# Chen-Suyi/PointRegGPT

Hardware: AMD Instinct MI355X
Metric: generated point-cloud pairs/sec (node), 128x128 depth, 1000-step DDNM (higher is better)
Workload: dtype bf16; 1 GPU; configs[2]: full pipeline (SE(3) z-buffer reproject + MaskUnet + DDNM sampler + MaskUnet + f64 unproject); batch_per_gpu=64, image_size=128, transitions=1000, sampler=ancestral-ddnm, unet_dim=64, streams=2, parallelism=scene-sharded x1, no collectives, hipgraph=one captured transition (U-Net + update), replayed per step

## Files before the change

### pointreggpt_amd/csrc/attn_fused.hip

```cpp
#include <atomic>
#include <cstdlib>
#include <type_traits>

#include "blocks.h"

namespace prg {

typedef __attribute__((ext_vector_type(8))) __bf16 bf16x8;
typedef __attribute__((ext_vector_type(16))) float f32x16;
typedef __attribute__((ext_vector_type(2))) float f32x2;

namespace {

constexpr int kTP = 64;
constexpr int kHid = 128;
constexpr int kTilesPerBlock = 8;
constexpr int kLaCtxTpb = 8, kLaOutTpb = 8;
__host__ __device__ inline int la_tpb(int ntiles) {
  const int t = ntiles / 8;
  return t < 1 ? 1 : (t > kLaCtxTpb ? kLaCtxTpb : t);
}
__host__ __device__ inline int la_out_tpb(int ntiles) {
  const int t = ntiles / 8;
  return t < 1 ? 1 : (t > kLaOutTpb ? kLaOutTpb : t);
}
constexpr int kLdO = kHid + 8;
constexpr float kLnEps = 1e-5f;

__device__ inline uint32_t pack2(float a, float b) {
  typedef __attribute__((ext_vector_type(2))) __bf16 bf16x2;
  bf16x2 v = {(__bf16)a, (__bf16)b};
  return __builtin_bit_cast(uint32_t, v);
}
__device__ inline float bf_lo(uint32_t w) { return __uint_as_float(w << 16); }
__device__ inline float bf_hi(uint32_t w) { return __uint_as_float(w & 0xffff0000u); }
__device__ inline float fast_exp(float x) { return __builtin_amdgcn_exp2f(x * 1.4426950408889634f); }

template <int C>
struct Geo {
  static constexpr int LDW = C + 8;
  static constexpr int VPT = C / 32;
  static constexpr int KK = C / 16;
};

__device__ inline float quad_sum(float v) {
  v += __builtin_bit_cast(float, __builtin_amdgcn_mov_dpp(__builtin_bit_cast(int, v), 0xB1, 0xF, 0xF, true));
  v += __builtin_bit_cast(float, __builtin_amdgcn_mov_dpp(__builtin_bit_cast(int, v), 0x4E, 0xF, 0xF, true));
  return v;
}

template <int C>
struct XTile {
  uint4 v[Geo<C>::VPT];
  __device__ inline void load(const bf16_t* x, int64_t pix0, int valid) {
    const int row = threadIdx.x >> 2, part = threadIdx.x & 3;
#pragma unroll
    for (int i = 0; i < Geo<C>::VPT; ++i)
      v[i] = row < valid ? *reinterpret_cast<const uint4*>(x + (pix0 + row) * C + (part + 4 * i) * 8) : make_uint4(0, 0, 0, 0);
  }
  __device__ inline void normalize_to(__bf16* xn) const {
    const int row = threadIdx.x >> 2, part = threadIdx.x & 3;
    float f[Geo<C>::VPT][8];
    float s = 0.0f;
#pragma unroll
    for (int i = 0; i < Geo<C>::VPT; ++i) {
      const uint32_t w[4] = {v[i].x, v[i].y, v[i].z, v[i].w};
#pragma unroll
      for (int j = 0; j < 4; ++j) {
        f[i][2 * j] = bf_lo(w[j]);
        f[i][2 * j + 1] = bf_hi(w[j]);
        s += f[i][2 * j] + f[i][2 * j + 1];
      }
    }
    s = quad_sum(s);
    const float mean = s * (1.0f / C);
    float q = 0.0f;
#pragma unroll
    for (int i = 0; i < Geo<C>::VPT; ++i)
#pragma unroll
      for (int j = 0; j < 8; ++j) {
        f[i][j] -= mean;
        q = fmaf(f[i][j], f[i][j], q);
      }
    q = quad_sum(q);
    const float rstd = __builtin_amdgcn_rsqf(q * (1.0f / C) + kLnEps);
#pragma unroll
    for (int i = 0; i < Geo<C>::VPT; ++i) {
      uint4 o;
      o.x = pack2(f[i][0] * rstd, f[i][1] * rstd);
      o.y = pack2(f[i][2] * rstd, f[i][3] * rstd);
      o.z = pack2(f[i][4] * rstd, f[i][5] * rstd);
      o.w = pack2(f[i][6] * rstd, f[i][7] * rstd);
      *reinterpret_cast<uint4*>(xn + row * Geo<C>::LDW + (part + 4 * i) * 8) = o;
    }
  }
};

template <int COLS, int LD>
__device__ inline void stage_rows(__bf16* dst, const bf16_t* src, int nrows) {
  constexpr int VR = COLS / 8;
  for (int i = threadIdx.x; i < nrows * VR; i += 256) {
    const int r = i / VR, v = i - r * VR;
    *reinterpret_cast<uint4*>(dst + r * LD + v * 8) = *reinterpret_cast<const uint4*>(src + (size_t)r * COLS + v * 8);
  }
}

__device__ inline bf16x8 frag(const __bf16* rows, int ld, int l31, int hi, int kk) {
  return *reinterpret_cast<const bf16x8*>(rows + l31 * ld + kk * 16 + hi * 8);
}

template <int COLS>
__device__ inline void load_wfrags(bf16x8 (&w)[COLS / 16], const bf16_t* mat, int r0, int l31, int hi) {
#pragma unroll
  for (int kk = 0; kk < COLS / 16; ++kk)
    w[kk] = *reinterpret_cast<const bf16x8*>(mat + (size_t)(r0 + l31) * COLS + kk * 16 + hi * 8);
}

__device__ inline f32x16 zero16() {
  f32x16 z;
#pragma unroll
  for (int e = 0; e < 16; ++e) z[e] = 0.0f;
  return z;
}

template <int C>
__global__ __launch_bounds__(256) void la_kmax_fused_kernel(const bf16_t* __restrict__ x, const bf16_t* __restrict__ wqkv,
                                                            float* __restrict__ pmax, int N, int nslab) {
  using G = Geo<C>;
  extern __shared__ __attribute__((aligned(16))) char smem[];
  __bf16* xn = reinterpret_cast<__bf16*>(smem);
  const int b = blockIdx.y, slab = blockIdx.x;
  const int wave = threadIdx.x >> 6, lane = threadIdx.x & 63, l31 = lane & 31, hi = lane >> 5;
  const int ntiles = (N + kTP - 1) / kTP;
  const int tpb = la_tpb(ntiles), t0 = slab * tpb, t1 = min(t0 + tpb, ntiles);
  bf16x8 wk[G::KK];
  load_wfrags<C>(wk, wqkv, kHid + 32 * wave, l31, hi);
  float m = -INFINITY;
  XTile<C> xt;
  if (t0 < t1) xt.load(x, (int64_t)b * N + (int64_t)t0 * kTP, min(kTP, N - t0 * kTP));
  for (int t = t0; t < t1; ++t) {
    xt.normalize_to(xn);
    __syncthreads();
    if (t + 1 < t1) xt.load(x, (int64_t)b * N + (int64_t)(t + 1) * kTP, min(kTP, N - (t + 1) * kTP));
    f32x16 acc[2] = {zero16(), zero16()};
#pragma unroll
    for (int kk = 0; kk < G::KK; ++kk) {
#pragma unroll
      for (int pt = 0; pt < 2; ++pt)
        acc[pt] = __builtin_amdgcn_mfma_f32_32x32x16_bf16(frag(xn + pt * 32 * G::LDW, G::LDW, l31, hi, kk), wk[kk], acc[pt], 0, 0, 0);
    }
    const int valid = min(kTP, N - t * kTP);
#pragma unroll
    for (int pt = 0; pt < 2; ++pt)
#pragma unroll
      for (int r = 0; r < 16; ++r) {
        const int px = pt * 32 + (r & 3) + 8 * (r >> 2) + 4 * hi;
        if (px < valid) m = fmaxf(m, acc[pt][r]);
      }
    __syncthreads();
  }
  m = fmaxf(m, __shfl_xor(m, 32, 64));
  if (hi == 0) pmax[((size_t)b * nslab + slab) * kHid + 32 * wave + l31] = m;
}

template <int C, bool PSUM_MFMA, bool KSTAT>
__global__ __launch_bounds__(256, C == 64 ? 3 : (C == 128 ? 2 : 1)) void la_ctx_fused_kernel(const bf16_t* __restrict__ x, const bf16_t* __restrict__ wqkv,
                                                           const float* __restrict__ pmax, float* __restrict__ ctxp,
                                                           float* __restrict__ sump, int N, int nslab) {
  using G = Geo<C>;
  extern __shared__ __attribute__((aligned(16))) char smem[];
  __bf16* xn = reinterpret_cast<__bf16*>(smem);
  const int b = blockIdx.y, slab = blockIdx.x;
  const int wave = threadIdx.x >> 6, lane = threadIdx.x & 63, l31 = lane & 31, hi = lane >> 5;
  const int ntiles = (N + kTP - 1) / kTP;
  const int tpb = la_tpb(ntiles), t0 = slab * tpb, t1 = min(t0 + tpb, ntiles);
  bf16x8 wk[G::KK], wv[G::KK];
  load_wfrags<C>(wk, wqkv, kHid + 32 * wave, l31, hi);
  load_wfrags<C>(wv, wqkv, 2 * kHid + 32 * wave, l31, hi);
  f32x16 kinit0 = zero16();
  if constexpr (!KSTAT) {
    float m = -INFINITY;
    for (int s2 = 0; s2 < nslab; ++s2) m = fmaxf(m, pmax[((size_t)b * nslab + s2) * kHid + 32 * wave + l31]);
#pragma unroll
    for (int e = 0; e < 16; ++e) kinit0[e] = -m;
  }
  f32x16 ctx = zero16();
  f32x16 psum = zero16();
  float ssum = 0.0f;
  bf16x8 ones;
#pragma unroll
  for (int e = 0; e < 8; ++e) ones[e] = (__bf16)1.0f;
  XTile<C> xt;
  if (t0 < t1) xt.load(x, (int64_t)b * N + (int64_t)t0 * kTP, min(kTP, N - t0 * kTP));
  for (int t = t0; t < t1; ++t) {
    xt.normalize_to(xn);
    __syncthreads();
    if (t + 1 < t1) xt.load(x, (int64_t)b * N + (int64_t)(t + 1) * kTP, min(kTP, N - (t + 1) * kTP));
    const int valid = min(kTP, N - t * kTP);
    auto half = [&](const int pt, auto full_c) {
      constexpr bool FULL = decltype(full_c)::value;
      f32x16 k1, v1;
#pragma unroll
      for (int kk = 0; kk < G::KK; ++kk) {
        const bf16x8 xf = frag(xn + pt * 32 * G::LDW, G::LDW, l31, hi, kk);
        k1 = __builtin_amdgcn_mfma_f32_32x32x16_bf16(xf, wk[kk], kk == 0 ? (KSTAT ? zero16() : kinit0) : k1, 0, 0, 0);
        v1 = __builtin_amdgcn_mfma_f32_32x32x16_bf16(xf, wv[kk], kk == 0 ? zero16() : v1, 0, 0, 0);
      }
#pragma unroll
      for (int i = 0; i < 2; ++i) {
        bf16x8 pa, vb;
#pragma unroll
        for (int s2 = 0; s2 < 8; ++s2) {
          const int r = 8 * i + s2;
          float pe = __builtin_amdgcn_exp2f(k1[r]);
          if constexpr (!FULL) pe = (pt * 32 + (r & 3) + 8 * (r >> 2) + 4 * hi) < valid ? pe : 0.0f;
          if constexpr (!PSUM_MFMA) ssum += pe;
          pa[s2] = (__bf16)pe;
          vb[s2] = (__bf16)v1[r];
        }
        ctx = __builtin_amdgcn_mfma_f32_32x32x16_bf16(pa, vb, ctx, 0, 0, 0);
        if constexpr (PSUM_MFMA) psum = __builtin_amdgcn_mfma_f32_32x32x16_bf16(pa, ones, psum, 0, 0, 0);
      }
    };
    if (valid == kTP) {
      half(0, std::true_type{});
      half(1, std::true_type{});
    } else {
      half(0, std::false_type{});
      half(1, std::false_type{});
    }
    __syncthreads();
  }
  const size_t ph = ((size_t)b * 4 + wave) * nslab + slab;
  if constexpr (PSUM_MFMA) {
    if (l31 == 0) {
#pragma unroll
      for (int r = 0; r < 16; ++r) sump[ph * 32 + (r & 3) + 8 * (r >> 2) + 4 * hi] = psum[r];
    }
  } else {
    ssum += __shfl_xor(ssum, 32, 64);
    if (hi == 0) sump[ph * 32 + l31] = ssum;
  }
#pragma unroll
  for (int r = 0; r < 16; ++r) ctxp[ph * 1024 + ((r & 3) + 8 * (r >> 2) + 4 * hi) * 32 + l31] = ctx[r];
}

__global__ __launch_bounds__(256) void la_fin_fused_kernel(const float* __restrict__ ctxp, const float* __restrict__ sump,
                                                           bf16_t* __restrict__ ctxT, int N, int nslab) {
  const int h = blockIdx.x, b = blockIdx.y;
  const size_t ph = ((size_t)b * 4 + h) * nslab;
  const float scale = 0.17677669529663687f / (float)N;
  for (int idx = threadIdx.x; idx < 1024; idx += 256) {
    const int d = idx >> 5, e = idx & 31;
    float c = 0.0f, s = 0.0f;
    int s2 = 0;
    for (; s2 + 8 <= nslab; s2 += 8) {
      float cv[8], sv[8];
#pragma unroll
      for (int u = 0; u < 8; ++u) {
        cv[u] = ctxp[(ph + s2 + u) * 1024 + idx];
        sv[u] = sump[(ph + s2 + u) * 32 + d];
      }
#pragma unroll
      for (int u = 0; u < 8; ++u) {
        c += cv[u];
        s += sv[u];
      }
    }
    for (; s2 < nslab; ++s2) {
      c += ctxp[(ph + s2) * 1024 + idx];
      s += sump[(ph + s2) * 32 + d];
    }
    const int slot = (d >> 4) * 16 + ((d >> 2) & 1) * 8 + ((d >> 3) & 1) * 4 + (d & 3);
    ctxT[((size_t)b * 4 + h) * 1024 + e * 32 + slot] = f32_to_bf16(c / s * scale);
  }
}

template <int C, bool QSTAT>
__global__ __launch_bounds__(256, C == 64 ? 3 : (C == 128 ? 2 : 1)) void la_out_fused_kernel(const bf16_t* __restrict__ x, const bf16_t* __restrict__ wqkv,
                                                           const bf16_t* __restrict__ wout, const float* __restrict__ bias,
                                                           const float* __restrict__ out_g, const bf16_t* __restrict__ ctxT,
                                                           bf16_t* __restrict__ out, int N, const float* __restrict__ qshift) {
  using G = Geo<C>;
  constexpr int RT = C / 32;
  constexpr int NA = RT / 2;
  constexpr int NR = RT > 4 ? RT / 4 : 1;
  constexpr int RTL = RT > 4 ? RT : 4;
  extern __shared__ __attribute__((aligned(16))) char smem[];
  __bf16* xn = reinterpret_cast<__bf16*>(smem);
  __bf16* ot = xn + kTP * G::LDW;
  float* lnb = reinterpret_cast<float*>(ot + kTP * kLdO);
  __bf16* yt = reinterpret_cast<__bf16*>(lnb + kTP * RTL * 2);
  float* bias_l = reinterpret_cast<float*>(yt + kTP * G::LDW);
  float* outg_l = bias_l + C;
  if (threadIdx.x < C) {
    bias_l[threadIdx.x] = bias[threadIdx.x];
    outg_l[threadIdx.x] = out_g[threadIdx.x];
  }
  const int b = blockIdx.y, slab = blockIdx.x;
  const int wave = threadIdx.x >> 6, lane = threadIdx.x & 63, l31 = lane & 31, hi = lane >> 5;
  const int ntiles = (N + kTP - 1) / kTP;
  const int tpb = la_out_tpb(ntiles), t0 = slab * tpb, t1 = min(t0 + tpb, ntiles);
  bf16x8 wq[G::KK];
  load_wfrags<C>(wq, wqkv, 32 * wave, l31, hi);
  bf16x8 ca[2];
#pragma unroll
  for (int i = 0; i < 2; ++i)
    ca[i] = *reinterpret_cast<const bf16x8*>(ctxT + (((size_t)b * 4 + wave) * 32 + l31) * 32 + i * 16 + hi * 8);
  int yrt[NA], ypt[NA];
#pragma unroll
  for (int a = 0; a < NA; ++a) {
    if (RT == 2) { yrt[a] = wave & 1; ypt[a] = wave >> 1; }
    else if (RT <= 4) { yrt[a] = wave; ypt[a] = a; }
    else { yrt[a] = wave * NR + (a >> 1); ypt[a] = a & 1; }
  }
  bf16x8 wo[NR][kHid / 16];
#pragma unroll
  for (int r = 0; r < NR; ++r) load_wfrags<kHid>(wo[r], wout, yrt[RT > 4 ? 2 * r : 0] * 32, l31, hi);
  XTile<C> xt;
  if (t0 < t1) xt.load(x, (int64_t)b * N + (int64_t)t0 * kTP, min(kTP, N - t0 * kTP));
  for (int t = t0; t < t1; ++t) {
    asm volatile("" ::: "memory");
    const XTile<C> xraw = xt;
    const int valid = min(kTP, N - t * kTP);
    xt.normalize_to(xn);
    __syncthreads();
    if (t + 1 < t1) xt.load(x, (int64_t)b * N + (int64_t)(t + 1) * kTP, min(kTP, N - (t + 1) * kTP));
    constexpr bool qstat = QSTAT;
    f32x16 qa[2];
#pragma unroll
    for (int kk = 0; kk < G::KK; ++kk) {
#pragma unroll
      for (int pt = 0; pt < 2; ++pt)
        qa[pt] = __builtin_amdgcn_mfma_f32_32x32x16_bf16(wq[kk], frag(xn + pt * 32 * G::LDW, G::LDW, l31, hi, kk),
                                                         kk == 0 ? zero16() : qa[pt], 0, 0, 0);
    }
#pragma unroll
    for (int pt = 0; pt < 2; ++pt) {
      f32x16 oa = zero16();
      if constexpr (qstat) {
        f32x16 sa = zero16();
        bf16x8 ones;
#pragma unroll
        for (int e = 0; e < 8; ++e) ones[e] = (__bf16)1.0f;
#pragma unroll
        for (int i = 0; i < 2; ++i) {
          bf16x8 qb;
#pragma unroll
          for (int s2 = 0; s2 < 8; ++s2) qb[s2] = (__bf16)__builtin_amdgcn_exp2f(qa[pt][8 * i + s2]);
          oa = __builtin_amdgcn_mfma_f32_32x32x16_bf16(ca[i], qb, oa, 0, 0, 0);
          sa = __builtin_amdgcn_mfma_f32_32x32x16_bf16(ones, qb, sa, 0, 0, 0);
        }
        const float inv = __builtin_amdgcn_rcpf(sa[0]);
        const f32x2 inv2 = {inv, inv};
#pragma unroll
        for (int r = 0; r < 16; r += 2) {
          const f32x2 o2 = f32x2{oa[r], oa[r + 1]} * inv2;
          oa[r] = o2[0];
          oa[r + 1] = o2[1];
        }
      } else {
        float mx = qa[pt][0];
#pragma unroll
        for (int r = 1; r < 16; ++r) mx = fmaxf(mx, qa[pt][r]);
        mx = fmaxf(mx, __shfl_xor(mx, 32, 64));
        float sm = 0.0f;
#pragma unroll
        for (int r = 0; r < 16; ++r) {
          qa[pt][r] = __builtin_amdgcn_exp2f(qa[pt][r] - mx);
          sm += qa[pt][r];
        }
        sm += __shfl_xor(sm, 32, 64);
        const float inv = 1.0f / sm;
#pragma unroll
        for (int i = 0; i < 2; ++i) {
          bf16x8 qb;
#pragma unroll
          for (int s2 = 0; s2 < 8; ++s2) qb[s2] = (__bf16)(qa[pt][8 * i + s2] * inv);
          oa = __builtin_amdgcn_mfma_f32_32x32x16_bf16(ca[i], qb, oa, 0, 0, 0);
        }
// ... 7 lines not shown
        *reinterpret_cast<uint2*>(ot + px * kLdO + 32 * wave + 8 * g4 + 4 * hi) = w;
      }
    }
    __syncthreads();
    f32x16 ya[NA];
#pragma unroll
    for (int a = 0; a < NA; ++a) ya[a] = zero16();
#pragma unroll
    for (int kk = 0; kk < kHid / 16; ++kk) {
#pragma unroll
      for (int a = 0; a < NA; ++a)
        ya[a] = __builtin_amdgcn_mfma_f32_32x32x16_bf16(wo[RT > 4 ? (a >> 1) : 0][kk],
                                                        frag(ot + ypt[a] * 32 * kLdO, kLdO, l31, hi, kk), ya[a], 0, 0, 0);
    }
#pragma unroll
    for (int a = 0; a < NA; ++a) {
      float s1 = 0.0f, s2 = 0.0f;
#pragma unroll
      for (int r = 0; r < 16; ++r) {
        const int c = yrt[a] * 32 + (r & 3) + 8 * (r >> 2) + 4 * hi;
        ya[a][r] += bias_l[c];
        s1 += ya[a][r];
        s2 = fmaf(ya[a][r], ya[a][r], s2);
      }
      const auto sw = __builtin_amdgcn_permlane32_swap(__builtin_bit_cast(unsigned, s1), __builtin_bit_cast(unsigned, s2), false, false);
      const float tot = __builtin_bit_cast(float, (unsigned)sw[0]) + __builtin_bit_cast(float, (unsigned)sw[1]);
      lnb[((ypt[a] * 32 + l31) * RTL + yrt[a]) * 2 + hi] = tot;
    }
    __syncthreads();
#pragma unroll
    for (int a = 0; a < NA; ++a) {
      const int px = ypt[a] * 32 + l31;
      float s1 = 0.0f, s2 = 0.0f;
#pragma unroll
      for (int rt = 0; rt < RT; ++rt) {
        s1 += lnb[(px * RTL + rt) * 2];
        s2 += lnb[(px * RTL + rt) * 2 + 1];
      }
      const float mean = s1 * (1.0f / C);
      const float rstd = __builtin_amdgcn_rsqf(fmaxf(s2 * (1.0f / C) - mean * mean, 0.0f) + kLnEps);
#pragma unroll
      for (int g4 = 0; g4 < 4; ++g4) {
        const int c0 = yrt[a] * 32 + 8 * g4 + 4 * hi;
        const float4 gg = *reinterpret_cast<const float4*>(outg_l + c0);
        uint2 w;
        w.x = pack2((ya[a][4 * g4] - mean) * rstd * gg.x, (ya[a][4 * g4 + 1] - mean) * rstd * gg.y);
        w.y = pack2((ya[a][4 * g4 + 2] - mean) * rstd * gg.z, (ya[a][4 * g4 + 3] - mean) * rstd * gg.w);
        *reinterpret_cast<uint2*>(yt + px * G::LDW + c0) = w;
      }
    }
    __syncthreads();
    {
      const int row = threadIdx.x >> 2, part = threadIdx.x & 3;
      if (row < valid) {
#pragma unroll
        for (int i = 0; i < G::VPT; ++i) {
          const uint4 yv = *reinterpret_cast<const uint4*>(yt + row * G::LDW + (part + 4 * i) * 8);
          const uint4 xv = xraw.v[i];
          uint4 o;
          o.x = pack2(bf_lo(yv.x) + bf_lo(xv.x), bf_hi(yv.x) + bf_hi(xv.x));
          o.y = pack2(bf_lo(yv.y) + bf_lo(xv.y), bf_hi(yv.y) + bf_hi(xv.y));
          o.z = pack2(bf_lo(yv.z) + bf_lo(xv.z), bf_hi(yv.z) + bf_hi(xv.z));
          o.w = pack2(bf_lo(yv.w) + bf_lo(xv.w), bf_hi(yv.w) + bf_hi(xv.w));
          *reinterpret_cast<uint4*>(out + ((int64_t)b * N + (int64_t)t * kTP + row) * C + (part + 4 * i) * 8) = o;
        }
      }
    }
  }
}

template <int NT>
__global__ __launch_bounds__(256) void full_attn_mfma_kernel(const bf16_t* __restrict__ qkv, bf16_t* __restrict__ out) {
  constexpr int N = 32 * NT, LDK = 40, LDV = N + 8;
  __shared__ __attribute__((aligned(16))) __bf16 Ks[N * LDK];
  __shared__ __attribute__((aligned(16))) __bf16 Vt[32 * LDV];
  const int h = blockIdx.x, b = blockIdx.y, tid = threadIdx.x;
  const int wave = tid >> 6, lane = tid & 63, l31 = lane & 31, hi = lane >> 5;
  const bf16_t* base = qkv + (size_t)b * N * 384;
  for (int i = tid; i < N * 4; i += 256) {
    const int key = i >> 2, u = i & 3;
    *reinterpret_cast<uint4*>(Ks + key * LDK + u * 8) =
        *reinterpret_cast<const uint4*>(base + (size_t)key * 384 + 128 + h * 32 + u * 8);
    const uint4 vv = *reinterpret_cast<const uint4*>(base + (size_t)key * 384 + 256 + h * 32 + u * 8);
    const int d = key & 31;
    const int pos = (key & ~31) + (d >> 4) * 16 + ((d >> 2) & 1) * 8 + ((d >> 3) & 1) * 4 + (d & 3);
    const uint32_t w[4] = {vv.x, vv.y, vv.z, vv.w};
#pragma unroll
    for (int j = 0; j < 4; ++j) {
      reinterpret_cast<uint16_t*>(Vt)[(u * 8 + 2 * j) * LDV + pos] = (uint16_t)(w[j] & 0xffffu);
      reinterpret_cast<uint16_t*>(Vt)[(u * 8 + 2 * j + 1) * LDV + pos] = (uint16_t)(w[j] >> 16);
    }
  }
  __syncthreads();
  for (int qt = wave; qt < NT; qt += 4) {
    const bf16_t* qp = base + (size_t)(qt * 32 + l31) * 384 + h * 32 + hi * 8;
    const bf16x8 q0 = *reinterpret_cast<const bf16x8*>(qp), q1 = *reinterpret_cast<const bf16x8*>(qp + 16);
    f32x16 sacc[NT];
    float m = -INFINITY;
#pragma unroll
    for (int kt = 0; kt < NT; ++kt) {
      sacc[kt] = zero16();
      sacc[kt] = __builtin_amdgcn_mfma_f32_32x32x16_bf16(frag(Ks + kt * 32 * LDK, LDK, l31, hi, 0), q0, sacc[kt], 0, 0, 0);
      sacc[kt] = __builtin_amdgcn_mfma_f32_32x32x16_bf16(frag(Ks + kt * 32 * LDK, LDK, l31, hi, 1), q1, sacc[kt], 0, 0, 0);
#pragma unroll
      for (int r = 0; r < 16; ++r) {
        sacc[kt][r] *= 0.17677669529663687f;
        m = fmaxf(m, sacc[kt][r]);
      }
    }
    m = fmaxf(m, __shfl_xor(m, 32, 64));
    float l = 0.0f;
    f32x16 oacc = zero16();
#pragma unroll
    for (int kt = 0; kt < NT; ++kt) {
#pragma unroll
      for (int i = 0; i < 2; ++i) {
        bf16x8 pb;
#pragma unroll
        for (int s2 = 0; s2 < 8; ++s2) {
          const float pv = fast_exp(sacc[kt][8 * i + s2] - m);
// ... 39 lines not shown
    for (int j = 0; j < 4; ++j) {
      reinterpret_cast<uint16_t*>(Vt)[(u * 8 + 2 * j) * LDV + pos] = (uint16_t)(w[j] & 0xffffu);
      reinterpret_cast<uint16_t*>(Vt)[(u * 8 + 2 * j + 1) * LDV + pos] = (uint16_t)(w[j] >> 16);
    }
  }
  __syncthreads();
  for (int qt = qs * 4 + wave; qt < NT; qt += 4 * QS) {
    const bf16_t* qp = base + (size_t)(qt * 32 + l31) * 384 + h * 32 + hi * 8;
    const bf16x8 q0 = *reinterpret_cast<const bf16x8*>(qp), q1 = *reinterpret_cast<const bf16x8*>(qp + 16);
    float m = -INFINITY;
#pragma unroll 2
    for (int kt = 0; kt < NT; ++kt) {
      f32x16 sa = zero16();
      sa = __builtin_amdgcn_mfma_f32_32x32x16_bf16(frag(Ks + kt * 32 * LDK, LDK, l31, hi, 0), q0, sa, 0, 0, 0);
      sa = __builtin_amdgcn_mfma_f32_32x32x16_bf16(frag(Ks + kt * 32 * LDK, LDK, l31, hi, 1), q1, sa, 0, 0, 0);
#pragma unroll
      for (int r = 0; r < 16; ++r) m = fmaxf(m, sa[r] * 0.17677669529663687f);
    }
    m = fmaxf(m, __shfl_xor(m, 32, 64));
    float l = 0.0f;
    f32x16 oacc = zero16();
#pragma unroll 2
    for (int kt = 0; kt < NT; ++kt) {
      f32x16 sa = zero16();
      sa = __builtin_amdgcn_mfma_f32_32x32x16_bf16(frag(Ks + kt * 32 * LDK, LDK, l31, hi, 0), q0, sa, 0, 0, 0);
      sa = __builtin_amdgcn_mfma_f32_32x32x16_bf16(frag(Ks + kt * 32 * LDK, LDK, l31, hi, 1), q1, sa, 0, 0, 0);
#pragma unroll
      for (int i = 0; i < 2; ++i) {
        bf16x8 pb;
#pragma unroll
        for (int s2 = 0; s2 < 8; ++s2) {
          const float pv = fast_exp(sa[8 * i + s2] * 0.17677669529663687f - m);
          l += pv;
          pb[s2] = (__bf16)pv;
        }
        oacc = __builtin_amdgcn_mfma_f32_32x32x16_bf16(
            *reinterpret_cast<const bf16x8*>(Vt + l31 * LDV + kt * 32 + i * 16 + hi * 8), pb, oacc, 0, 0, 0);
      }
    }
    l += __shfl_xor(l, 32, 64);
    const float inv = 1.0f / l;
    bf16_t* op = out + ((size_t)b * N + qt * 32 + l31) * 128 + h * 32 + 4 * hi;
#pragma unroll
    for (int g4 = 0; g4 < 4; ++g4) {
      uint2 w;
      w.x = pack2(oacc[4 * g4] * inv, oacc[4 * g4 + 1] * inv);
      w.y = pack2(oacc[4 * g4 + 2] * inv, oacc[4 * g4 + 3] * inv);
      *reinterpret_cast<uint2*>(op + 8 * g4) = w;
    }
  }
}

template <int C>
size_t lds_kmax() { return (size_t)kTP * Geo<C>::LDW * 2; }
template <int C>
size_t lds_out() { return (size_t)2 * kTP * Geo<C>::LDW * 2 + (size_t)kTP * kLdO * 2 + (size_t)kTP * (C / 32 > 4 ? C / 32 : 4) * 2 * 4 + (size_t)2 * C * 4; }

template <typename K>
int set_lds(K kernel, size_t bytes) {
  hipError_t e = hipFuncSetAttribute(reinterpret_cast<const void*>(kernel), hipFuncAttributeMaxDynamicSharedMemorySize, (int)bytes);
  if (e != hipSuccess) return fail(PRG_E_HIP, std::string("hipFuncSetAttribute(fused attention): ") + hipGetErrorString(e));
  return PRG_OK;
}

int la_slabs(int N) { const int nt = ceil_div(N, kTP); return ceil_div(nt, la_tpb(nt)); }
int tail_slabs(int N) { return ceil_div(ceil_div(N, kTP), kTilesPerBlock); }

constexpr int kTailDepth = 2;
template <int CIN, int COUT>
__global__ __launch_bounds__(256, COUT == 64 ? 3 : 2) void resblock_tail_fused_kernel(
    const bf16_t* __restrict__ h, const float* __restrict__ A, const float* __restrict__ Bc, const bf16_t* __restrict__ s0, int C0,
    const bf16_t* __restrict__ s1, int C1, const bf16_t* __restrict__ wres, const float* __restrict__ bres, bf16_t* __restrict__ out,
    int N, const float* __restrict__ head_w, const float* __restrict__ head_b, float* __restrict__ head_out, int head_sigmoid,
    const GnFold fold) {
  constexpr int LDX = CIN + 8, LDH = COUT + 8;
  constexpr int RT = COUT / 32, NA = RT / 2;
  constexpr int XV = CIN / 32, HV = COUT / 32;
  extern __shared__ __attribute__((aligned(16))) char smem[];
  __bf16* xs = reinterpret_cast<__bf16*>(smem);
  __bf16* hs = xs + kTP * LDX;
  float* cf = reinterpret_cast<float*>(hs + kTP * LDH);
  const int b = blockIdx.y, slab = blockIdx.x;
  const int wave = threadIdx.x >> 6, lane = threadIdx.x & 63, l31 = lane & 31, hi = lane >> 5;
  const int row = threadIdx.x >> 2, part = threadIdx.x & 3;
  const int ntiles = (N + kTP - 1) / kTP;
  const int t0 = slab * kTilesPerBlock, t1 = min(t0 + kTilesPerBlock, ntiles);
  const int yrt = RT == 2 ? (wave & 1) : wave;
  int ypt[NA];
#pragma unroll
  for (int a = 0; a < NA; ++a) ypt[a] = RT == 2 ? (wave >> 1) : a;
  bf16x8 wr[CIN / 16];
  load_wfrags<CIN>(wr, wres, yrt * 32, l31, hi);
  if (threadIdx.x < COUT) {
    const int c = threadIdx.x;
    float a, bb;
    if (fold.acc) {
      float mean, rstd;
      gn_fold_stats(fold, b, c / fold.cpg, mean, rstd);
      a = rstd * fold.P[(size_t)b * fold.pq_stride + c];
      bb = fmaf(-mean, a, fold.Q[(size_t)b * fold.pq_stride + c]);
    } else {
      a = A[(size_t)b * COUT + c];
      bb = Bc[(size_t)b * COUT + c];
    }
    cf[c] = a;
    cf[COUT + c] = bb;
    cf[2 * COUT + c] = bres[c];
// ... 64 lines not shown
          acc = fmaf(bf_hi(q[j]), w[2 * j + 1], acc);
        }
      }
      acc += __shfl_xor(acc, 1, 64);
      acc += __shfl_xor(acc, 2, 64);
      if (part == 0 && row < valid) {
        const float y = acc + hb;
        head_out[(int64_t)b * N + (int64_t)t * kTP + row] = head_sigmoid ? 1.0f / (1.0f + expf(-y)) : y;
      }
    } else if (row < valid) {
#pragma unroll
      for (int i = 0; i < HV; ++i)
        *reinterpret_cast<uint4*>(out + ((int64_t)b * N + (int64_t)t * kTP + row) * COUT + (part + 4 * i) * 8) =
            *reinterpret_cast<const uint4*>(hs + row * LDH + (part + 4 * i) * 8);
    }
    __syncthreads();
  };
  load_tile(ta, t0);
  load_tile(tb, t0 + 1);
  for (int t = t0; t < t1; t += kTailDepth) {
    do_tile(ta, t);
    do_tile(tb, t + 1);
  }
}

template <int CIN, int COUT>
int launch_tail(const bf16_t* h, const float* A, const float* Bc, const bf16_t* s0, int C0, const bf16_t* s1, int C1,
                const bf16_t* wres, const float* bres, bf16_t* out, int B, int N, hipStream_t s, const GnFold& fold,
                const float* head_w = nullptr, const float* head_b = nullptr, float* head_out = nullptr, int head_sigmoid = 0) {
  const size_t lds = (size_t)kTP * (CIN + 8 + COUT + 8) * 2 + (size_t)4 * COUT * 4;
  static DeviceOnce attr;
  if (!attr.done()) {
    int rc = set_lds(&resblock_tail_fused_kernel<CIN, COUT>, lds);
    if (rc) return rc;
    attr.mark();
  }
  resblock_tail_fused_kernel<CIN, COUT><<<dim3(tail_slabs(N), B), 256, lds, s>>>(h, A, Bc, s0, C0, s1, C1, wres, bres, out, N, head_w, head_b,
                                                                                 head_out, head_sigmoid, fold);
  PRG_LAUNCH_CHECK();
  return PRG_OK;
}


template <int C>
constexpr bool kPsumDefault = C >= 128;

template <int C>
int launch_c(const bf16_t* x, const bf16_t* wqkv, const bf16_t* wout, const float* bias, const float* out_g, bf16_t* out,
             float* ws, int B, int N, const float* kshift, hipStream_t s, int psum_override) {
  static DeviceOnce attr;
  if (!attr.done()) {
    int rc;
    if ((rc = set_lds(&la_kmax_fused_kernel<C>, lds_kmax<C>()))) return rc;
    if ((rc = set_lds(&la_ctx_fused_kernel<C, false, false>, lds_kmax<C>()))) return rc;
    if ((rc = set_lds(&la_ctx_fused_kernel<C, false, true>, lds_kmax<C>()))) return rc;
    if ((rc = set_lds(&la_ctx_fused_kernel<C, true, false>, lds_kmax<C>()))) return rc;
    if ((rc = set_lds(&la_ctx_fused_kernel<C, true, true>, lds_kmax<C>()))) return rc;
    if ((rc = set_lds(&la_out_fused_kernel<C, false>, lds_out<C>()))) return rc;
    if ((rc = set_lds(&la_out_fused_kernel<C, true>, lds_out<C>()))) return rc;
    attr.mark();
  }
  const int nslab = la_slabs(N);
  float* pmax = ws;
  float* ctxp = pmax + (size_t)B * nslab * kHid;
  float* sump = ctxp + (size_t)B * 4 * nslab * 1024;
  bf16_t* ctxT = reinterpret_cast<bf16_t*>(sump + (size_t)B * 4 * nslab * 32);
  const dim3 grid(nslab, B);
  if (!kshift) {
    la_kmax_fused_kernel<C><<<grid, 256, lds_kmax<C>(), s>>>(x, wqkv, pmax, N, nslab);
    PRG_LAUNCH_CHECK();
  }
  static const int psum_env = env_int("PRG_LA_PSUM", -1);
  const int psum_sel = psum_override >= 0 ? psum_override : psum_env;
  const bool psum = psum_sel > 0 || (psum_sel < 0 && kPsumDefault<C>);
#define PRG_LA_CTX_GO(PS, KS) la_ctx_fused_kernel<C, PS, KS><<<grid, 256, lds_kmax<C>(), s>>>(x, wqkv, pmax, ctxp, sump, N, nslab)
  if (kshift) { if (psum) PRG_LA_CTX_GO(true, true); else PRG_LA_CTX_GO(false, true); }
  else { if (psum) PRG_LA_CTX_GO(true, false); else PRG_LA_CTX_GO(false, false); }
#undef PRG_LA_CTX_GO
  PRG_LAUNCH_CHECK();
  la_fin_fused_kernel<<<dim3(4, B), 256, 0, s>>>(ctxp, sump, ctxT, N, nslab);
  PRG_LAUNCH_CHECK();
  const int nt = ceil_div(N, kTP);
  const dim3 ogrid(ceil_div(nt, la_out_tpb(nt)), B);
  if (kshift) la_out_fused_kernel<C, true><<<ogrid, 256, lds_out<C>(), s>>>(x, wqkv, wout, bias, out_g, ctxT, out, N, kshift + kHid);
  else la_out_fused_kernel<C, false><<<ogrid, 256, lds_out<C>(), s>>>(x, wqkv, wout, bias, out_g, ctxT, out, N, nullptr);
  PRG_LAUNCH_CHECK();
  return PRG_OK;
}

}

bool full_attention_mfma_supported(int N) { return N == 64 || N == 128 || N == 256 || N == 512 || N == 1024; }

template <int NT, int QS>
static int launch_attn_big(const bf16_t* qkv, bf16_t* out, int B, hipStream_t s) {
  constexpr int N = 32 * NT;
  constexpr size_t lds = ((size_t)N * 40 + (size_t)32 * (N + 8)) * 2;
  static DeviceOnce attr;
  if (!attr.done()) {
    int rc = set_lds(&full_attn_mfma_big_kernel<NT, QS>, lds);
    if (rc) return rc;
    attr.mark();
  }
  full_attn_mfma_big_kernel<NT, QS><<<dim3(4, B, QS), 256, lds, s>>>(qkv, out);
  PRG_LAUNCH_CHECK();
  return PRG_OK;
}

int launch_full_attention_mfma(const bf16_t* qkv, bf16_t* out, int B, int N, hipStream_t s) {
  PRG_CHECK(full_attention_mfma_supported(N) && qkv && out, "full attention (MFMA): unsupported token count");
  const dim3 grid(4, B);
  if (N == 1024) return B >= 32 ? launch_attn_big<32, 2>(qkv, out, B, s) : launch_attn_big<32, 4>(qkv, out, B, s);
  if (N == 512) return launch_attn_big<16, 2>(qkv, out, B, s);
  if (N == 64) full_attn_mfma_kernel<2><<<grid, 256, 0, s>>>(qkv, out);
  else if (N == 128) full_attn_mfma_kernel<4><<<grid, 256, 0, s>>>(qkv, out);
  else full_attn_mfma_kernel<8><<<grid, 256, 0, s>>>(qkv, out);
  PRG_LAUNCH_CHECK();
  return PRG_OK;
}

bool resblock_tail_fused_supported(int C0, int C1, int Cout) {
  const int cin = C0 + C1;
  return C0 % 8 == 0 && C1 % 8 == 0 && ((cin == 128 && Cout == 64) || (cin == 192 && Cout == 128) || (cin == 256 && Cout == 128));
}

int launch_resblock_tail_fused(const bf16_t* h, const float* A, const float* Bc, const bf16_t* s0, int C0, const bf16_t* s1,
                               int C1, const bf16_t* wres, const float* bres, bf16_t* out, int B, int N, int Cout,
                               hipStream_t s,
// ... 34 lines not shown
```

Measured before the change: 14.90 pairs/s.

## Software-pipeline linear-attention context kernel with double-buffered LDS and pinned MFMA/VALU schedule

For C<=128, the linear-attention context kernel gets double-buffered LDS tiles. The loop is restructured so the K/V projection MFMA chain for the next half-tile runs while the exp2 and bf16 packing of the previous half run on the VALU. sched_group_barrier pinning and s_setprio interleave the MFMA, DS-read and VALU groups, and one barrier per tile replaces the two __syncthreads. This costs double the LDS per block, which can lower occupancy, and adds more complex scheduling code with a tail epilogue.

```diff
diff --git a/pointreggpt_amd/csrc/attn_fused.hip b/pointreggpt_amd/csrc/attn_fused.hip
--- a/pointreggpt_amd/csrc/attn_fused.hip
+++ b/pointreggpt_amd/csrc/attn_fused.hip
@@ -114,6 +114,29 @@
 #pragma unroll
   for (int kk = 0; kk < COLS / 16; ++kk)
     w[kk] = *reinterpret_cast<const bf16x8*>(mat + (size_t)(r0 + l31) * COLS + kk * 16 + hi * 8);
+}
+
+__device__ inline void lds_barrier() {
+  asm volatile("s_waitcnt lgkmcnt(0)" ::: "memory");
+  __builtin_amdgcn_s_barrier();
+  asm volatile("" ::: "memory");
+}
+
+template <int NG, int G, int TR, int VA>
+__device__ inline void pin_groups() {
+  if constexpr (NG > 0) {
+    __builtin_amdgcn_sched_group_barrier(0x008, G, 0);
+    __builtin_amdgcn_sched_group_barrier(0x400, TR, 0);
+    __builtin_amdgcn_sched_group_barrier(0x002, VA, 0);
+    pin_groups<NG - 1, G, TR, VA>();
+  }
+}
+template <int DSR, int NG, int G, int TR, int VA>
+__device__ inline void pin_chain_under_valu() {
+  __builtin_amdgcn_sched_group_barrier(0x100, DSR, 0);
+  __builtin_amdgcn_sched_group_barrier(0x400, TR, 0);
+  __builtin_amdgcn_sched_group_barrier(0x002, VA, 0);
+  pin_groups<NG, G, TR, VA>();
 }
 
 __device__ inline f32x16 zero16() {
@@ -163,7 +186,7 @@
   if (hi == 0) pmax[((size_t)b * nslab + slab) * kHid + 32 * wave + l31] = m;
 }
 
-template <int C, bool PSUM_MFMA, bool KSTAT>
+template <int C, bool PSUM_MFMA, bool KSTAT, bool PIPE>
 __global__ __launch_bounds__(256, C == 64 ? 3 : (C == 128 ? 2 : 1)) void la_ctx_fused_kernel(const bf16_t* __restrict__ x, const bf16_t* __restrict__ wqkv,
                                                            const float* __restrict__ pmax, float* __restrict__ ctxp,
                                                            float* __restrict__ sump, int N, int nslab) {
@@ -191,45 +214,116 @@
 #pragma unroll
   for (int e = 0; e < 8; ++e) ones[e] = (__bf16)1.0f;
   XTile<C> xt;
-  if (t0 < t1) xt.load(x, (int64_t)b * N + (int64_t)t0 * kTP, min(kTP, N - t0 * kTP));
-  for (int t = t0; t < t1; ++t) {
-    xt.normalize_to(xn);
-    __syncthreads();
-    if (t + 1 < t1) xt.load(x, (int64_t)b * N + (int64_t)(t + 1) * kTP, min(kTP, N - (t + 1) * kTP));
-    const int valid = min(kTP, N - t * kTP);
-    auto half = [&](const int pt, auto full_c) {
-      constexpr bool FULL = decltype(full_c)::value;
-      f32x16 k1, v1;
+  if constexpr (PIPE) {
+    const int64_t img = (int64_t)b * N;
+    auto load_x = [&](int t) { xt.load(x, img + (int64_t)t * kTP, min(kTP, N - t * kTP)); };
+    auto chain = [&](const __bf16* buf, const int pt, f32x16& k1, f32x16& v1) {
 #pragma unroll
       for (int kk = 0; kk < G::KK; ++kk) {
-        const bf16x8 xf = frag(xn + pt * 32 * G::LDW, G::LDW, l31, hi, kk);
+        const bf16x8 xf = frag(buf + pt * 32 * G::LDW, G::LDW, l31, hi, kk);
         k1 = __builtin_amdgcn_mfma_f32_32x32x16_bf16(xf, wk[kk], kk == 0 ? (KSTAT ? zero16() : kinit0) : k1, 0, 0, 0);
         v1 = __builtin_amdgcn_mfma_f32_32x32x16_bf16(xf, wv[kk], kk == 0 ? zero16() : v1, 0, 0, 0);
       }
-#pragma unroll
-      for (int i = 0; i < 2; ++i) {
-        bf16x8 pa, vb;
+    };
+    auto exps = [&](const f32x16& k1, const f32x16& v1, const int pt, const int valid, auto full_c, bf16x8 (&pa)[2], bf16x8 (&vb)[2]) {
+      constexpr bool FULL = decltype(full_c)::value;
+#pragma unroll
+      for (int i = 0; i < 2; ++i)
 #pragma unroll
         for (int s2 = 0; s2 < 8; ++s2) {
           const int r = 8 * i + s2;
           float pe = __builtin_amdgcn_exp2f(k1[r]);
           if constexpr (!FULL) pe = (pt * 32 + (r & 3) + 8 * (r >> 2) + 4 * hi) < valid ? pe : 0.0f;
           if constexpr (!PSUM_MFMA) ssum += pe;
-          pa[s2] = (__bf16)pe;
-          vb[s2] = (__bf16)v1[r];
-        }
-        ctx = __builtin_amdgcn_mfma_f32_32x32x16_bf16(pa, vb, ctx, 0, 0, 0);
-        if constexpr (PSUM_MFMA) psum = __builtin_amdgcn_mfma_f32_32x32x16_bf16(pa, ones, psum, 0, 0, 0);
-      }
+          pa[i][s2] = (__bf16)pe;
+          vb[i][s2] = (__bf16)v1[r];
+        }
     };
-    if (valid == kTP) {
-      half(0, std::true_type{});
-      half(1, std::true_type{});
-    } else {
-      half(0, std::false_type{});
-      half(1, std::false_type{});
-    }
-    __syncthreads();
+    auto accum = [&](const bf16x8 (&pa)[2], const bf16x8 (&vb)[2]) {
+#pragma unroll
+      for (int i = 0; i < 2; ++i) {
+        ctx = __builtin_amdgcn_mfma_f32_32x32x16_bf16(pa[i], vb[i], ctx, 0, 0, 0);
+        if constexpr (PSUM_MFMA) psum = __builtin_amdgcn_mfma_f32_32x32x16_bf16(pa[i], ones, psum, 0, 0, 0);
+      }
+    };
+    if (t0 < t1) {
+      __bf16* cur = xn;
+      __bf16* nxt = xn + kTP * G::LDW;
+      f32x16 kA, vA, kB, vB;
+      bf16x8 pa[2], vb[2], pb[2], wb[2];
+      load_x(t0);
+      xt.normalize_to(cur);
+      if (t0 + 1 < t1) load_x(t0 + 1);
+      lds_barrier();
+      chain(cur, 0, kA, vA);
+      for (int t = t0; t + 1 < t1; ++t) {
+        __builtin_amdgcn_s_setprio(2);
+        chain(cur, 1, kB, vB);
+        exps(kA, vA, 0, kTP, std::true_type{}, pa, vb);
+        pin_chain_under_valu<G::KK, 8, G::KK / 4, 2, 3>();
+        accum(pa, vb);
+        __builtin_amdgcn_s_setprio(0);
+        xt.normalize_to(nxt);
+        if (t + 2 < t1) load_x(t + 2);
+        lds_barrier();
+        __builtin_amdgcn_s_setprio(2);
+        chain(nxt, 0, kA, vA);
+        exps(kB, vB, 1, kTP, std::true_type{}, pb, wb);
+        pin_chain_under_valu<G::KK, 8, G::KK / 4, 2, 3>();
+        accum(pb, wb);
+        __builtin_amdgcn_s_setprio(0);
+        __bf16* const sw = cur;
+        cur = nxt;
+        nxt = sw;
+      }
+      const int valid = min(kTP, N - (t1 - 1) * kTP);
+      chain(cur, 1, kB, vB);
+      exps(kA, vA, 0, valid, std::false_type{}, pa, vb);
+      accum(pa, vb);
+      exps(kB, vB, 1, valid, std::false_type{}, pb, wb);
+      accum(pb, wb);
+    }
+  } else {
+    if (t0 < t1) xt.load(x, (int64_t)b * N + (int64_t)t0 * kTP, min(kTP, N - t0 * kTP));
+    for (int t = t0; t < t1; ++t) {
+      xt.normalize_to(xn);
+      __syncthreads();
+      if (t + 1 < t1) xt.load(x, (int64_t)b * N + (int64_t)(t + 1) * kTP, min(kTP, N - (t + 1) * kTP));
+      const int valid = min(kTP, N - t * kTP);
+      auto half = [&](const int pt, auto full_c) {
+        constexpr bool FULL = decltype(full_c)::value;
+        f32x16 k1, v1;
+#pragma unroll
+        for (int kk = 0; kk < G::KK; ++kk) {
+          const bf16x8 xf = frag(xn + pt * 32 * G::LDW, G::LDW, l31, hi, kk);
+          k1 = __builtin_amdgcn_mfma_f32_32x32x16_bf16(xf, wk[kk], kk == 0 ? (KSTAT ? zero16() : kinit0) : k1, 0, 0, 0);
+          v1 = __builtin_amdgcn_mfma_f32_32x32x16_bf16(xf, wv[kk], kk == 0 ? zero16() : v1, 0, 0, 0);
+        }
+#pragma unroll
+        for (int i = 0; i < 2; ++i) {
+          bf16x8 pa, vb;
+#pragma unroll
+          for (int s2 = 0; s2 < 8; ++s2) {
+            const int r = 8 * i + s2;
+            float pe = __builtin_amdgcn_exp2f(k1[r]);
+            if constexpr (!FULL) pe = (pt * 32 + (r & 3) + 8 * (r >> 2) + 4 * hi) < valid ? pe : 0.0f;
+            if constexpr (!PSUM_MFMA) ssum += pe;
+            pa[s2] = (__bf16)pe;
+            vb[s2] = (__bf16)v1[r];
+          }
+          ctx = __builtin_amdgcn_mfma_f32_32x32x16_bf16(pa, vb, ctx, 0, 0, 0);
+          if constexpr (PSUM_MFMA) psum = __builtin_amdgcn_mfma_f32_32x32x16_bf16(pa, ones, psum, 0, 0, 0);
+        }
+      };
+      if (valid == kTP) {
+        half(0, std::true_type{});
+        half(1, std::true_type{});
+      } else {
+        half(0, std::false_type{});
+        half(1, std::false_type{});
+      }
+      __syncthreads();
+    }
   }
   const size_t ph = ((size_t)b * 4 + wave) * nslab + slab;
   if constexpr (PSUM_MFMA) {
@@ -598,7 +692,12 @@
 }
 
 template <int C>
+constexpr bool kCtxPipe = C <= 128;
+
+template <int C>
 size_t lds_kmax() { return (size_t)kTP * Geo<C>::LDW * 2; }
+template <int C>
+size_t lds_ctx() { return (kCtxPipe<C> ? 2 : 1) * lds_kmax<C>(); }
 template <int C>
 size_t lds_out() { return (size_t)2 * kTP * Geo<C>::LDW * 2 + (size_t)kTP * kLdO * 2 + (size_t)kTP * (C / 32 > 4 ? C / 32 : 4) * 2 * 4 + (size_t)2 * C * 4; }
 
@@ -769,10 +868,10 @@
   if (!attr.done()) {
     int rc;
     if ((rc = set_lds(&la_kmax_fused_kernel<C>, lds_kmax<C>()))) return rc;
-    if ((rc = set_lds(&la_ctx_fused_kernel<C, false, false>, lds_kmax<C>()))) return rc;
-    if ((rc = set_lds(&la_ctx_fused_kernel<C, false, true>, lds_kmax<C>()))) return rc;
-    if ((rc = set_lds(&la_ctx_fused_kernel<C, true, false>, lds_kmax<C>()))) return rc;
-    if ((rc = set_lds(&la_ctx_fused_kernel<C, true, true>, lds_kmax<C>()))) return rc;
+    if ((rc = set_lds(&la_ctx_fused_kernel<C, false, false, kCtxPipe<C>>, lds_ctx<C>()))) return rc;
+    if ((rc = set_lds(&la_ctx_fused_kernel<C, false, true, kCtxPipe<C>>, lds_ctx<C>()))) return rc;
+    if ((rc = set_lds(&la_ctx_fused_kernel<C, true, false, kCtxPipe<C>>, lds_ctx<C>()))) return rc;
+    if ((rc = set_lds(&la_ctx_fused_kernel<C, true, true, kCtxPipe<C>>, lds_ctx<C>()))) return rc;
     if ((rc = set_lds(&la_out_fused_kernel<C, false>, lds_out<C>()))) return rc;
     if ((rc = set_lds(&la_out_fused_kernel<C, true>, lds_out<C>()))) return rc;
     attr.mark();
@@ -790,7 +889,7 @@
   static const int psum_env = env_int("PRG_LA_PSUM", -1);
   const int psum_sel = psum_override >= 0 ? psum_override : psum_env;
   const bool psum = psum_sel > 0 || (psum_sel < 0 && kPsumDefault<C>);
-#define PRG_LA_CTX_GO(PS, KS) la_ctx_fused_kernel<C, PS, KS><<<grid, 256, lds_kmax<C>(), s>>>(x, wqkv, pmax, ctxp, sump, N, nslab)
+#define PRG_LA_CTX_GO(PS, KS) la_ctx_fused_kernel<C, PS, KS, kCtxPipe<C>><<<grid, 256, lds_ctx<C>(), s>>>(x, wqkv, pmax, ctxp, sump, N, nslab)
   if (kshift) { if (psum) PRG_LA_CTX_GO(true, true); else PRG_LA_CTX_GO(false, true); }
   else { if (psum) PRG_LA_CTX_GO(true, false); else PRG_LA_CTX_GO(false, false); }
 #undef PRG_LA_CTX_GO
```

Result: no change. 14.88 pairs/s (-0.1%).

## Double-tile ctx loop for C=64 and split full/tail tiles in linear attention

Applied to the files above, without the earlier changes.

For C=64 the linear-attention context kernel now normalizes two 64-pixel tiles per iteration into a doubled LDS buffer, with two prefetch registers, so each pair of barriers covers four MFMA halves. Full tiles and the tail tile are separated so the common path drops per-row validity checks and uses unconditional loads. The output kernel gets a clamped, branch-free prefetch and a FULL-specialised store. The aim is fewer barriers and less predication per tile, at the cost of more LDS and more registers for C=64, which may lower occupancy.

```diff
diff --git a/pointreggpt_amd/csrc/attn_fused.hip b/pointreggpt_amd/csrc/attn_fused.hip
--- a/pointreggpt_amd/csrc/attn_fused.hip
+++ b/pointreggpt_amd/csrc/attn_fused.hip
@@ -52,14 +52,20 @@
 template <int C>
 struct XTile {
   uint4 v[Geo<C>::VPT];
+  __device__ static inline int own_row() { return threadIdx.x >> 2; }
   __device__ inline void load(const bf16_t* x, int64_t pix0, int valid) {
-    const int row = threadIdx.x >> 2, part = threadIdx.x & 3;
+    const int row = own_row(), part = threadIdx.x & 3;
 #pragma unroll
     for (int i = 0; i < Geo<C>::VPT; ++i)
       v[i] = row < valid ? *reinterpret_cast<const uint4*>(x + (pix0 + row) * C + (part + 4 * i) * 8) : make_uint4(0, 0, 0, 0);
   }
+  __device__ inline void load_full(const bf16_t* x, int64_t pix0, int row = own_row()) {
+    const int part = threadIdx.x & 3;
+#pragma unroll
+    for (int i = 0; i < Geo<C>::VPT; ++i) v[i] = *reinterpret_cast<const uint4*>(x + (pix0 + row) * C + (part + 4 * i) * 8);
+  }
   __device__ inline void normalize_to(__bf16* xn) const {
-    const int row = threadIdx.x >> 2, part = threadIdx.x & 3;
+    const int row = own_row(), part = threadIdx.x & 3;
     float f[Geo<C>::VPT][8];
     float s = 0.0f;
 #pragma unroll
@@ -69,7 +75,9 @@
       for (int j = 0; j < 4; ++j) {
         f[i][2 * j] = bf_lo(w[j]);
         f[i][2 * j + 1] = bf_hi(w[j]);
-        s += f[i][2 * j] + f[i][2 * j + 1];
+        float pr = f[i][2 * j] + f[i][2 * j + 1];
+        asm("" : "+v"(pr));
+        s += pr;
       }
     }
     s = quad_sum(s);
@@ -190,46 +198,96 @@
   bf16x8 ones;
 #pragma unroll
   for (int e = 0; e < 8; ++e) ones[e] = (__bf16)1.0f;
-  XTile<C> xt;
-  if (t0 < t1) xt.load(x, (int64_t)b * N + (int64_t)t0 * kTP, min(kTP, N - t0 * kTP));
-  for (int t = t0; t < t1; ++t) {
-    xt.normalize_to(xn);
-    __syncthreads();
-    if (t + 1 < t1) xt.load(x, (int64_t)b * N + (int64_t)(t + 1) * kTP, min(kTP, N - (t + 1) * kTP));
-    const int valid = min(kTP, N - t * kTP);
-    auto half = [&](const int pt, auto full_c) {
-      constexpr bool FULL = decltype(full_c)::value;
-      f32x16 k1, v1;
+  auto half = [&](const __bf16* rows, auto full_c, const int px0, const int valid) {
+    constexpr bool FULL = decltype(full_c)::value;
+    f32x16 k1, v1;
+    if constexpr (C == 64) {
+      bf16x8 xf[G::KK];
+#pragma unroll
+      for (int kk = 0; kk < G::KK; ++kk) xf[kk] = frag(rows, G::LDW, l31, hi, kk);
 #pragma unroll
       for (int kk = 0; kk < G::KK; ++kk) {
-        const bf16x8 xf = frag(xn + pt * 32 * G::LDW, G::LDW, l31, hi, kk);
+        k1 = __builtin_amdgcn_mfma_f32_32x32x16_bf16(xf[kk], wk[kk], kk == 0 ? (KSTAT ? zero16() : kinit0) : k1, 0, 0, 0);
+        v1 = __builtin_amdgcn_mfma_f32_32x32x16_bf16(xf[kk], wv[kk], kk == 0 ? zero16() : v1, 0, 0, 0);
+      }
+    } else {
+#pragma unroll
+      for (int kk = 0; kk < G::KK; ++kk) {
+        const bf16x8 xf = frag(rows, G::LDW, l31, hi, kk);
         k1 = __builtin_amdgcn_mfma_f32_32x32x16_bf16(xf, wk[kk], kk == 0 ? (KSTAT ? zero16() : kinit0) : k1, 0, 0, 0);
         v1 = __builtin_amdgcn_mfma_f32_32x32x16_bf16(xf, wv[kk], kk == 0 ? zero16() : v1, 0, 0, 0);
       }
-#pragma unroll
-      for (int i = 0; i < 2; ++i) {
-        bf16x8 pa, vb;
-#pragma unroll
-        for (int s2 = 0; s2 < 8; ++s2) {
-          const int r = 8 * i + s2;
-          float pe = __builtin_amdgcn_exp2f(k1[r]);
-          if constexpr (!FULL) pe = (pt * 32 + (r & 3) + 8 * (r >> 2) + 4 * hi) < valid ? pe : 0.0f;
-          if constexpr (!PSUM_MFMA) ssum += pe;
-          pa[s2] = (__bf16)pe;
-          vb[s2] = (__bf16)v1[r];
-        }
-        ctx = __builtin_amdgcn_mfma_f32_32x32x16_bf16(pa, vb, ctx, 0, 0, 0);
-        if constexpr (PSUM_MFMA) psum = __builtin_amdgcn_mfma_f32_32x32x16_bf16(pa, ones, psum, 0, 0, 0);
-      }
-    };
-    if (valid == kTP) {
-      half(0, std::true_type{});
-      half(1, std::true_type{});
-    } else {
-      half(0, std::false_type{});
-      half(1, std::false_type{});
-    }
-    __syncthreads();
+    }
+#pragma unroll
+    for (int i = 0; i < 2; ++i) {
+      bf16x8 pa, vb;
+#pragma unroll
+      for (int s2 = 0; s2 < 8; ++s2) {
+        const int r = 8 * i + s2;
+        float pe = __builtin_amdgcn_exp2f(k1[r]);
+        if constexpr (!FULL) pe = (px0 + (r & 3) + 8 * (r >> 2) + 4 * hi) < valid ? pe : 0.0f;
+        if constexpr (!PSUM_MFMA) ssum += pe;
+        pa[s2] = (__bf16)pe;
+        vb[s2] = (__bf16)v1[r];
+      }
+      ctx = __builtin_amdgcn_mfma_f32_32x32x16_bf16(pa, vb, ctx, 0, 0, 0);
+      if constexpr (PSUM_MFMA) psum = __builtin_amdgcn_mfma_f32_32x32x16_bf16(pa, ones, psum, 0, 0, 0);
+    }
+  };
+  const int tfull = min(t1, N / kTP);
+  const int64_t img = (int64_t)b * N;
+  auto fetch = [&](XTile<C>& xt, int t) {
+    if (t < tfull) xt.load_full(x, img + (int64_t)t * kTP);
+    else if (t < t1) xt.load(x, img + (int64_t)t * kTP, N - t * kTP);
+  };
+  XTile<C> xt;
+  fetch(xt, t0);
+  int t = t0;
+  if constexpr (C == 64) {
+    XTile<C> xu;
+    fetch(xu, t0 + 1);
+    for (; t + 2 <= tfull; t += 2) {
+      xt.normalize_to(xn);
+      xu.normalize_to(xn + kTP * G::LDW);
+      __syncthreads();
+      fetch(xt, t + 2);
+      fetch(xu, t + 3);
+#pragma unroll
+      for (int h4 = 0; h4 < 4; ++h4) half(xn + h4 * 32 * G::LDW, std::true_type{}, 0, 0);
+      __syncthreads();
+    }
+    if (t < t1) {
+      const int left = t1 - t;
+      xt.normalize_to(xn);
+      if (left == 2) xu.normalize_to(xn + kTP * G::LDW);
+      __syncthreads();
+      if (t < tfull) {
+        half(xn, std::true_type{}, 0, 0);
+        half(xn + 32 * G::LDW, std::true_type{}, 0, 0);
+      }
+      if (tfull < t1) {
+        const __bf16* rows = xn + (tfull - t) * kTP * G::LDW;
+        const int valid = N - tfull * kTP;
+        half(rows, std::false_type{}, 0, valid);
+        half(rows + 32 * G::LDW, std::false_type{}, 32, valid);
+      }
+    }
+  } else {
+    for (; t < tfull; ++t) {
+      xt.normalize_to(xn);
+      __syncthreads();
+      fetch(xt, t + 1);
+      half(xn, std::true_type{}, 0, 0);
+      half(xn + 32 * G::LDW, std::true_type{}, 0, 0);
+      __syncthreads();
+    }
+    if (t < t1) {
+      const int valid = N - t * kTP;
+      xt.normalize_to(xn);
+      __syncthreads();
+      half(xn, std::false_type{}, 0, valid);
+      half(xn + 32 * G::LDW, std::false_type{}, 32, valid);
+    }
   }
   const size_t ph = ((size_t)b * 4 + wave) * nslab + slab;
   if constexpr (PSUM_MFMA) {
@@ -318,14 +376,20 @@
 #pragma unroll
   for (int r = 0; r < NR; ++r) load_wfrags<kHid>(wo[r], wout, yrt[RT > 4 ? 2 * r : 0] * 32, l31, hi);
   XTile<C> xt;
-  if (t0 < t1) xt.load(x, (int64_t)b * N + (int64_t)t0 * kTP, min(kTP, N - t0 * kTP));
-  for (int t = t0; t < t1; ++t) {
+  constexpr bool COUNTED = C == 64;
+  const int plast = min(t1 * kTP, N) - 1;
+  auto fetch = [&](int t) {
+    if constexpr (COUNTED) xt.load_full(x, (int64_t)b * N, min(t * kTP + XTile<C>::own_row(), plast));
+    else if (t < t1) xt.load(x, (int64_t)b * N + (int64_t)t * kTP, min(kTP, N - t * kTP));
+  };
+  auto tile = [&](const int t, auto full_c) {
+    constexpr bool FULL = decltype(full_c)::value;
     asm volatile("" ::: "memory");
     const XTile<C> xraw = xt;
     const int valid = min(kTP, N - t * kTP);
     xt.normalize_to(xn);
     __syncthreads();
-    if (t + 1 < t1) xt.load(x, (int64_t)b * N + (int64_t)(t + 1) * kTP, min(kTP, N - (t + 1) * kTP));
+    fetch(t + 1);
     constexpr bool qstat = QSTAT;
     f32x16 qa[2];
 #pragma unroll
@@ -439,7 +503,7 @@
     __syncthreads();
     {
       const int row = threadIdx.x >> 2, part = threadIdx.x & 3;
-      if (row < valid) {
+      if (FULL || row < valid) {
 #pragma unroll
         for (int i = 0; i < G::VPT; ++i) {
           const uint4 yv = *reinterpret_cast<const uint4*>(yt + row * G::LDW + (part + 4 * i) * 8);
@@ -453,6 +517,18 @@
         }
       }
     }
+  };
+  fetch(t0);
+  if constexpr (COUNTED) {
+    const int tfull = min(t1, N / kTP);
+    int t = t0;
+    if (t < tfull) {
+      tile(t, std::true_type{});
+      for (++t; t < tfull; ++t) tile(t, std::true_type{});
+    }
+    if (t < t1) tile(t, std::false_type{});
+  } else {
+    for (int t = t0; t < t1; ++t) tile(t, std::false_type{});
   }
 }
 
@@ -599,6 +675,8 @@
 
 template <int C>
 size_t lds_kmax() { return (size_t)kTP * Geo<C>::LDW * 2; }
+template <int C>
+size_t lds_ctx() { return (size_t)(C == 64 ? 2 : 1) * kTP * Geo<C>::LDW * 2; }
 template <int C>
 size_t lds_out() { return (size_t)2 * kTP * Geo<C>::LDW * 2 + (size_t)kTP * kLdO * 2 + (size_t)kTP * (C / 32 > 4 ? C / 32 : 4) * 2 * 4 + (size_t)2 * C * 4; }
 
@@ -769,10 +847,10 @@
   if (!attr.done()) {
     int rc;
     if ((rc = set_lds(&la_kmax_fused_kernel<C>, lds_kmax<C>()))) return rc;
-    if ((rc = set_lds(&la_ctx_fused_kernel<C, false, false>, lds_kmax<C>()))) return rc;
-    if ((rc = set_lds(&la_ctx_fused_kernel<C, false, true>, lds_kmax<C>()))) return rc;
-    if ((rc = set_lds(&la_ctx_fused_kernel<C, true, false>, lds_kmax<C>()))) return rc;
-    if ((rc = set_lds(&la_ctx_fused_kernel<C, true, true>, lds_kmax<C>()))) return rc;
+    if ((rc = set_lds(&la_ctx_fused_kernel<C, false, false>, lds_ctx<C>()))) return rc;
+    if ((rc = set_lds(&la_ctx_fused_kernel<C, false, true>, lds_ctx<C>()))) return rc;
+    if ((rc = set_lds(&la_ctx_fused_kernel<C, true, false>, lds_ctx<C>()))) return rc;
+    if ((rc = set_lds(&la_ctx_fused_kernel<C, true, true>, lds_ctx<C>()))) return rc;
     if ((rc = set_lds(&la_out_fused_kernel<C, false>, lds_out<C>()))) return rc;
     if ((rc = set_lds(&la_out_fused_kernel<C, true>, lds_out<C>()))) return rc;
     attr.mark();
@@ -790,7 +868,7 @@
   static const int psum_env = env_int("PRG_LA_PSUM", -1);
   const int psum_sel = psum_override >= 0 ? psum_override : psum_env;
   const bool psum = psum_sel > 0 || (psum_sel < 0 && kPsumDefault<C>);
-#define PRG_LA_CTX_GO(PS, KS) la_ctx_fused_kernel<C, PS, KS><<<grid, 256, lds_kmax<C>(), s>>>(x, wqkv, pmax, ctxp, sump, N, nslab)
+#define PRG_LA_CTX_GO(PS, KS) la_ctx_fused_kernel<C, PS, KS><<<grid, 256, lds_ctx<C>(), s>>>(x, wqkv, pmax, ctxp, sump, N, nslab)
   if (kshift) { if (psum) PRG_LA_CTX_GO(true, true); else PRG_LA_CTX_GO(false, true); }
   else { if (psum) PRG_LA_CTX_GO(true, false); else PRG_LA_CTX_GO(false, false); }
 #undef PRG_LA_CTX_GO
```

Result: no change. 14.33 pairs/s before, 14.31 pairs/s after (-0.2%).
